# withterm/term

Hardware: AMD Instinct MI355X
Metric: validated rows/sec, 16-col null+range+unique suite (higher is better)
Workload: dtype int64+f64; 1 GPU; 16-col (8 int64 + 8 float64, 12 nullable) null+range+unique suite: completeness x16, min/max/mean x16, uniqueness x2; rows_total=1000000000, rows_per_gpu=1000000000, cols=16, parallelism=row-range shards x1, HSA_ENABLE_IPC_MODE_LEGACY=0, suite_algorithmic_bytes=129500000000, verified=True

## Files before the change

### term_amd/csrc/distinct_state.cpp

```cpp
#include "api_internal.h"

tgx_status distinct_read_counters(tgx_state *st, DistinctState &ds, unsigned long long *out,
                                         tgx_error *err) {
  memset(out, 0, kNumDistinctCounters * sizeof(unsigned long long));
  if (!ds.counters.p) return TGX_OK;
  HIP_TRY(hipMemcpyAsync(out, ds.counters.p, kNumDistinctCounters * sizeof(unsigned long long),
                         hipMemcpyDeviceToHost, st->stream));
  HIP_TRY(hipStreamSynchronize(st->stream));
  return TGX_OK;
}

tgx_status pinned_readback(tgx_state *st, size_t bytes, tgx_error *err) {
  if (bytes <= st->h_pinned_cap) return TGX_OK;
  pinned_free(st->h_pinned, st->h_pinned_cap);
  st->h_pinned = nullptr;
  st->h_pinned_cap = 0;
  const size_t want = std::max<size_t>(bytes + bytes / 2, 4096);
  HIP_TRY(pinned_alloc(&st->h_pinned, want));
  st->h_pinned_cap = want;
  return TGX_OK;
}

namespace {

// ... 587 lines not shown
        ds.range = top - (uint64_t)base + 1;
        use_bitmap = true;
      }
    }
    if (use_bitmap) {
      size_t words = (size_t)(((ds.range + (1u << 20) - 1) >> 20) << 15) + 4;
      ds.bitmap_words = words - 4;
      if (ds.seen.cap < words * 4 && ds.spare_seen.cap >= words * 4) std::swap(ds.seen, ds.spare_seen);
      if (ds.twice.cap < words * 4 && ds.spare_twice.cap >= words * 4) std::swap(ds.twice, ds.spare_twice);
      HIP_TRY(ds.seen.reserve(words * 4));
      HIP_TRY(hipMemsetAsync(ds.seen.p, 0, words * 4, st->stream));
      if (mult) {
        HIP_TRY(ds.twice.reserve(words * 4));
        HIP_TRY(hipMemsetAsync(ds.twice.p, 0, words * 4, st->stream));
      }
      ds.mode = DistinctMode::kBitmap;
      ds.speculative = !ds.has_hint;
      if (ds.speculative && !facts.range_known) {
        ds.remembered = true;
        ds.remembered_lo = lo;
        ds.remembered_hi = hi;
      }
    } else {
      ds.mode = DistinctMode::kHash;
      ds.remembered = false;
    }
  }
  if (ds.mode == DistinctMode::kBitmap && ds.speculative && !ds.partitioned && facts.range_known &&
      !ds.outliers_possible)
    TGX_TRY(bitmap_grow(st, ds, mult, facts.lo, facts.hi, c.length, err));
  if (ds.mode == DistinctMode::kBitmap && ds.speculative) {
    auto u = [](int64_t v) { return (uint64_t)v ^ 0x8000000000000000ull; };
    const bool covered = facts.range_known && u(facts.lo) >= u(ds.base) && u(facts.hi) - u(ds.base) < ds.range;
    if (!covered) ds.outliers_possible = true;
  }
  if (ds.mode == DistinctMode::kBitmap) {
    bitmap_shape(ds, c.length, mult, &prep->sub_bits, &prep->key16, &prep->n_buckets, &prep->partitioned);
    if (ds.partitioned) prep->partitioned = false;
  }
  return TGX_OK;
}

namespace {

tgx_status distinct_run_numeric(tgx_state *st, size_t slot, const tgx_column &c, const NumericPrep &prep,
                                       int stats_slot, tgx_error *err, const tgx_column *orig) {
  const DistinctTask &task = st->plan->distinct[slot];
  const tgx_column &keep = (orig && orig->mem == TGX_MEM_DEVICE && is_widened(orig->type)) ? *orig : c;
  DistinctState &ds = st->distinct[slot];
  const bool mult = task.multiplicity;
  const DistinctColDesc d = numeric_desc(c, mult);
  const uint64_t bytes = (uint64_t)c.length * 8 + (c.validity ? (uint64_t)(c.length + 7) / 8 : 0);
  if (ds.mode == DistinctMode::kUndecided) return TGX_OK;
  if (ds.mode == DistinctMode::kBitmap) {
    if (ds.speculative) ds.retained.push_back(keep);
    if (prep.partitioned) {
      PartitionParams pp;
      memset(&pp, 0, sizeof(pp));
      pp.values = c.values;
      pp.validity = c.validity;
      pp.offset = c.offset;
      pp.length = c.length;
      pp.base = ds.base;
      pp.range = ds.range;
      pp.sub_bits = prep.sub_bits;
      pp.n_buckets = (uint32_t)prep.n_buckets;
      const uint64_t tiles = ((uint64_t)c.length + kPartitionTile - 1) / kPartitionTile;
      pp.bucket0 = 0;
      pp.n_lists = pp.n_buckets;
      if (prep.range_known) {
        auto u = [](int64_t v) { return (uint64_t)v ^ 0x8000000000000000ull; };
        const uint64_t ub = u(ds.base);
        const uint64_t rlo = u(prep.lo) > ub ? u(prep.lo) - ub : 0;
        uint64_t rhi = u(prep.hi) > ub ? u(prep.hi) - ub : 0;
        rhi = std::min(rhi, ds.range - 1);
        if (rlo <= rhi) {
          pp.bucket0 = (uint32_t)(rlo >> pp.sub_bits);
          pp.n_lists = (uint32_t)(rhi >> pp.sub_bits) - pp.bucket0 + 1;
        }
      }
      const char *p20 = getenv("TGX_PACK20");
      const bool no_pack20 = p20 && atoi(p20) == 0;
      const bool pack20 = !prep.key16 && prep.sub_bits <= (mult ? 19u : 20u) && !no_pack20;
      uint64_t cap = (uint64_t)c.length / pp.n_lists;
      cap = cap + cap / 4 + (prep.key16 ? 32 : pack20 ? 24 : 16) * tiles + 4096;
      pp.cap = prep.key16 ? (cap + 31) & ~31ull : pack20 ? (cap + 23) / 24 * 24 : (cap + 15) & ~15ull;
      if (pp.cap >= (1ull << 32) - 64) return fail(err, TGX_INTERNAL, "distinct: list capacity out of range");
      pp.want_multiplicity = mult ? 1 : 0;
      pp.key16 = prep.key16 ? 1 : pack20 ? 2 : 0;
      pp.force_form = ds.remembered_form;
      HIP_TRY(ds.lists.reserve(prep.key16 ? (uint64_t)pp.n_lists * pp.cap * sizeof(uint16_t)
                               : pack20   ? (uint64_t)pp.n_lists * pp.cap / 3 * 8
                                          : (uint64_t)pp.n_lists * pp.cap * sizeof(uint32_t)));
      HIP_TRY(ds.cursors.reserve((2 * pp.n_buckets + 1) * sizeof(unsigned long long)));
      pp.lists = ds.lists.as<uint32_t>();
      pp.cursors = ds.cursors.as<unsigned long long>();
      pp.seen = ds.seen.as<uint32_t>();
      pp.twice = mult ? ds.twice.as<uint32_t>() : nullptr;
      const int grid = partition_grid(c.length, g_ctx.n_cu);
      if (stats_slot >= 0) {
        HIP_TRY(ds.stat_partials.reserve((size_t)(grid + 1) * sizeof(ScanPartial)));
        HIP_TRY(ds.outlier_stats.reserve(sizeof(OutlierStats)));
        pp.stats = ds.stat_partials.as<ScanPartial>();
        pp.outliers = ds.outlier_stats.as<OutlierStats>();
      }
      unsigned long long *cnt = ds.counters.as<unsigned long long>();
      static_assert(kCntDistinct == 0 && kCntTwice == 1, "partition_init_kernel clears the two totals together");
      launch_partition_init(pp, cnt + kCntDistinct, st->stream);
      {
        ProfScope ps(st, "distinct", bytes);
        launch_partition(pp, cnt, g_ctx.n_cu, st->stream);
        HIP_TRY(launch_bucket_apply(pp, cnt, st->stream));
      }
      if (stats_slot >= 0) {
        ScanLaunch L;
        memset(&L, 0, sizeof(L));
        L.cols[0].length = c.length;
        L.cols[0].is_float = 0;
        L.acc_index[0] = stats_slot;
        launch_scan_reduce_only(L, 1, grid, pp.stats, st->d_scan_acc.as<ScanAcc>(), st->stream, pp.outliers);
      }
    } else {
      ProfScope ps(st, "distinct", bytes);
      launch_distinct_bitmap(d, bitmap_view(ds), ds.counters.as<unsigned long long>(), st->stream);
    }
  } else {
    if (ds.fp_staged) TGX_TRY(distinct_resolve(st, slot, err));
    if (ds.capacity == 0 && fp_lists_fit(c)) {
      FpLists l1, l2;
      uint32_t *fb_lo = nullptr;
      TGX_TRY(fp_lists_stage(st, ds, c.length, false, &l1, &l2, &fb_lo, err));
      ProfScope ps(st, "distinct", bytes), ps_lists(st, "distinct_lists", 0);
      launch_key_lists(d, l1, l2, mult ? 1 : 0, ds.fp_per_list.as<uint2>(), ds.counters.as<unsigned long long>(),
                       st->stream);
      ds.retained.push_back(keep);
      return TGX_OK;
    }
    TGX_TRY(hash_ensure(st, ds, mult, (uint64_t)c.length, err));
    ProfScope ps(st, "distinct", bytes);
    launch_distinct_hash(d, hash_view(ds), ds.counters.as<unsigned long long>(), st->stream);
  }
  return TGX_OK;
}

tgx_status retained_numeric_view(tgx_state *st, const tgx_column &col, std::vector<std::unique_ptr<DevBuf>> &tmp,
                                        tgx_column *out, tgx_error *err) {
  *out = col;
  if (!is_widened(col.type)) return TGX_OK;
  const int64_t e0 = col.offset & ~(int64_t)63;
  const int64_t slots = col.offset - e0 + col.length;
  tmp.emplace_back(new DevBuf());
  DevBuf *w = tmp.back().get();
  HIP_TRY(w->reserve((size_t)slots * 8 + 16));
  launch_widen32((const uint8_t *)col.values + narrow_bytes(col.type, e0), w->p, slots, widen_mode(col.type), g_ctx.n_cu,
                 st->stream);
  out->type = widened_type(col.type);
  out->values = w->p;
  out->validity = col.validity ? col.validity + (e0 >> 3) : nullptr;
  out->offset = col.offset - e0;
  return TGX_OK;
}

}

tgx_status distinct_update(tgx_state *st, size_t slot, const tgx_column &c, const BatchKeyFacts &facts,
                           const NumericPrep &prep, tgx_error *err, const std::vector<DictGather> *gathers,
                           int stats_slot, const tgx_column *orig) {
  const DistinctTask &task = st->plan->distinct[slot];
// ... 515 lines not shown
```

### term_amd/csrc/kernels/distinct_types.h

```cpp
#pragma once
#include <stdint.h>

namespace tgx {

constexpr uint64_t kEmptyKey = 0xFFFFFFFFFFFFFFFFULL;

struct DistinctColDesc {
  const void *values;
  const uint8_t *validity;
  int64_t offset;
  int64_t length;
  int32_t want_multiplicity;
  int32_t pad;
};

struct HashSetView {
  uint64_t *keys;
  uint32_t *dup;
  uint64_t mask;
  uint64_t *store;
  unsigned long long *store_cursor;
  uint64_t store_words;
  uint64_t *pending;
  uint32_t *pending_counts;
  uint64_t pending_region;
  uint32_t pending_waves, pad_;
};
inline uint32_t exact_blocks(uint64_t items) {
  uint64_t blocks = (items + 255) / 256;
  if (blocks < 1) blocks = 1;
  if (blocks > 2048) blocks = 2048;
  return (uint32_t)blocks;
}
inline uint32_t exact_waves(uint64_t items) { return exact_blocks(items) * 4; }
inline uint64_t exact_region(uint64_t items) {
  const uint64_t threads = (uint64_t)exact_blocks(items) * 256;
  return (items + threads - 1) / threads * 64;
}

struct FpKey {
  uint32_t k[4], k1[4], k2[4];
};
inline void fp_key_times_two(const uint32_t in[4], uint32_t out[4]) {
  const uint32_t carry = (in[3] >> 31) ? 0x87u : 0u;
  out[3] = (in[3] << 1) | (in[2] >> 31);
  out[2] = (in[2] << 1) | (in[1] >> 31);
  out[1] = (in[1] << 1) | (in[0] >> 31);
  out[0] = (in[0] << 1) ^ carry;
}
inline FpKey fp_key_expand(const uint32_t k[4]) {
  FpKey key;
  for (int i = 0; i < 4; i++) key.k[i] = k[i];
  fp_key_times_two(key.k, key.k1);
  fp_key_times_two(key.k1, key.k2);
  return key;
}

struct Utf8ColDesc {
  const void *offsets;
  const uint8_t *data;
  const uint8_t *validity;
  int64_t offset;
  int64_t length;
  int32_t large_offsets;
  int32_t want_multiplicity;
  const void *views;
  const uint8_t *const *buffers;
  FpKey key;
};

struct BitmapView {
  uint32_t *seen;
  uint32_t *twice;
  int64_t base;
  uint64_t range;
};

constexpr uint32_t kMaxPartitions = 2048;
constexpr uint32_t kListPad = 0xFFFFFFFFu;
constexpr int kRunPad4 = 16, kRunPad2 = 32;
constexpr int kPartitionThreads = 1024;
constexpr int kPartitionKeysPerThread = 32;
constexpr int kPartitionTile = kPartitionThreads * kPartitionKeysPerThread;
constexpr int kSliceWordsLds = 32768;

struct PartitionParams {
  const void *values;
  const uint8_t *validity;
  int64_t offset;
  int64_t length;
  int64_t base;
  uint64_t range;
  uint32_t sub_bits;
  uint32_t n_buckets;
  uint64_t cap;
  uint32_t *lists;
  unsigned long long *cursors;
  uint32_t *seen;
  uint32_t *twice;
  int32_t want_multiplicity;
  int32_t key16;
  struct ScanPartial *stats;
  struct OutlierStats *outliers;
  uint32_t bucket0, n_lists;
  int32_t force_form;
};

struct OutlierStats {
  long long mn, mx;
  unsigned long long lo32_sum;
  long long hi32_sum;
  unsigned long long count;
};

struct DistinctSample {
  int64_t min_v, max_v;
  unsigned long long count;
  unsigned long long pad;
};

struct KeyRecord {
  uint64_t key;
  uint64_t count;
};

struct KeyRecord128 {
  uint64_t a, b;
  uint64_t count;
  uint64_t pad;
};

constexpr int kFpFan = 256;
constexpr int kFpXcds = 8;
constexpr int kFpTile = 2048;
constexpr uint32_t kFpSlots = 4096;
constexpr uint32_t kFpListMax = 24576;
constexpr int64_t kFpMinRows = 1 << 21;
struct FpLists {
  uint64_t *recs;
  uint32_t *offered;
  uint64_t cap;
};

enum {
  kCntDistinct = 0,
  kCntTwice = 1,
  kCntEmptyRows = 2,
  kCntValidRows = 3,
  kCntOutOfRange = 4,
  kCntSpare = 5,
  kCntStoreFull = 6,
  kCntForm = 7,
  kNumDistinctCounters = 8
};

struct TupleCol {
  int32_t kind;
  int32_t dict_large;
  const void *values;
  const void *offsets;
  const uint8_t *data;
  const uint8_t *const *buffers;
  const uint8_t *validity;
  int64_t offset;
  const uint8_t *dict_validity;
  int64_t dict_offset;
};
constexpr int kMaxTupleCols = 8;
struct TupleDesc {
  TupleCol cols[kMaxTupleCols];
  int32_t n_cols;
  int32_t want_multiplicity;
  int64_t length;
  FpKey key;
};

}
```

### term_amd/csrc/kernels/partition.hip

```cpp
#include <hip/hip_runtime.h>

#include <type_traits>

#include "device_types.h"
#include "distinct_types.h"
#include "keyset_device.h"

namespace tgx {

template <int THREADS, int KPT, bool VALIDITY>
__device__ __forceinline__ void partition_load_tile(const PartitionParams &p, int64_t tile, bool wide,
                                                    int64_t (&key)[KPT], uint32_t &ok) {
  constexpr int kPartitionThreads = THREADS;
  constexpr int kTile = kPartitionThreads * KPT;
  global_i64_ptr vals = (global_i64_ptr)(uintptr_t)((const int64_t *)p.values + p.offset);
  global_u8_ptr vbits = VALIDITY ? (global_u8_ptr)(uintptr_t)p.validity : (global_u8_ptr) nullptr;
  const uint32_t tid = threadIdx.x;
  const int64_t row0 = tile * kTile;
  const bool full = row0 + kTile <= p.length;
  ok = 0;
  if (full && wide) {
    typedef long long i64x2 __attribute__((ext_vector_type(2)));
    typedef const i64x2 __attribute__((address_space(1))) *global_i64x2_ptr;
    global_i64x2_ptr pv = (global_i64x2_ptr)(vals + row0) + tid;
    const bool pair_bytes = vbits && (p.offset & 1) == 0;
    ok = (uint32_t)((1ull << KPT) - 1ull);
    if (pair_bytes) {
      uint8_t vb[KPT / 2];
#pragma unroll
      for (int j = 0; j < KPT / 2; j++) {
        const int64_t bit = p.offset + row0 + (int64_t)j * 2 * kPartitionThreads + 2 * tid;
        vb[j] = vbits[bit >> 3];
      }
      ok = 0;
#pragma unroll
      for (int j = 0; j < KPT / 2; j++) {
        const int64_t bit = p.offset + row0 + (int64_t)j * 2 * kPartitionThreads + 2 * tid;
        ok |= (uint32_t)((vb[j] >> (bit & 7)) & 3) << (2 * j);
      }
    } else if (vbits) {
      ok = 0;
#pragma unroll
      for (int j = 0; j < KPT; j++) {
        const int64_t bit = p.offset + row0 + (int64_t)(j / 2) * 2 * kPartitionThreads + 2 * tid + (j & 1);
        ok |= (uint32_t)TGX_VALID_BIT(vbits, bit) << j;
      }
    }
    if (VALIDITY) asm volatile("" : "+v"(ok));
#pragma unroll
    for (int j = 0; j < KPT / 2; j++) {
      i64x2 v = pv[(int64_t)j * kPartitionThreads];
      key[2 * j] = v.x;
      key[2 * j + 1] = v.y;
    }
  } else {
#pragma unroll
    for (int j = 0; j < KPT; j++) {
      const int64_t i = row0 + (int64_t)j * kPartitionThreads + tid;
      const bool in = i < p.length;
      key[j] = vals[in ? i : p.length - 1];
      bool valid = in;
      if (in && vbits) {
        const int64_t bit = p.offset + i;
        valid = TGX_VALID_BIT(vbits, bit);
      }
      ok |= (uint32_t)valid << j;
    }
  }
}

template <int THREADS, int KPT, int MAXP, int PAD, bool KEY16, bool PACK20, bool CLUSTERED, class MidFn, class StoreFn>
__device__ __forceinline__ void partition_process_tile(const PartitionParams &p, uint32_t *sorted, uint32_t *hist,
                                                       uint32_t *toff, uint32_t *gbase, uint32_t *wave_sums,
                                                       uint32_t *long_runs, const uint32_t (&rel)[KPT], uint64_t ok,
                                                       MidFn &&mid,
                                                       StoreFn &&before_stores) {
  constexpr uint32_t NW = THREADS / 64;
  constexpr int BPT = MAXP / THREADS;
  constexpr int NS = MAXP / (NW * 64);
  static_assert(MAXP % THREADS == 0 && MAXP % (NW * 64) == 0 && PAD % 4 == 0, "shape");
  constexpr uint32_t RPAD = PACK20 ? 24u : KEY16 ? (uint32_t)kRunPad2 : (uint32_t)PAD;
  auto pad_up = [](uint32_t h) -> uint32_t { return PACK20 ? (h + 23u) / 24u * 24u : (h + (RPAD - 1u)) & ~(RPAD - 1u); };
  const bool fill = p.want_multiplicity != 0;
  auto pack6 = [&](uint32_t o, uint32_t h, uint32_t i) -> uint4 {
    uint64_t w[2];
    if (!fill) {
#pragma unroll
      for (int q = 0; q < 2; q++) {
        const uint32_t i0 = i + 3u * q;
        const uint64_t a = sorted[o + (i0 < h ? i0 : h - 1)], b = sorted[o + (i0 + 1 < h ? i0 + 1 : h - 1)],
                       c = sorted[o + (i0 + 2 < h ? i0 + 2 : h - 1)];
        w[q] = a | (b << 20) | (c << 40);
      }
    } else {
#pragma unroll
      for (int q = 0; q < 2; q++) {
        uint64_t e[3];
#pragma unroll
        for (uint32_t j = 0; j < 3; j++) {
          const uint32_t at = i + 3u * q + j;
          e[j] = at < h ? (uint64_t)sorted[o + at] : 0xFFFFFull;
        }
        w[q] = e[0] | (e[1] << 20) | (e[2] << 40);
      }
    }
    return make_uint4((uint32_t)w[0], (uint32_t)(w[0] >> 32), (uint32_t)w[1], (uint32_t)(w[1] >> 32));
  };
  const uint32_t tid = threadIdx.x;
  const uint32_t lane = tid & 63, wave = tid >> 6;
  const uint32_t sub_mask = (uint32_t)((1ull << p.sub_bits) - 1);
  for (uint32_t b = tid; b < (uint32_t)MAXP; b += THREADS) hist[b] = 0;
  constexpr uint32_t kLongRun = 1024, kMaxLongRuns = THREADS * KPT / kLongRun;
  if (CLUSTERED && tid == 0) long_runs[kMaxLongRuns] = 0;
  __syncthreads();
  bool whole = false;
  if (CLUSTERED) {
    uint32_t agreed = 0;
#pragma unroll
    for (int j = 0; j < KPT; j++) {
      const bool okj = (ok >> j) & 1;
      const uint32_t b = rel[j] >> p.sub_bits;
      const uint64_t act = __ballot(okj);
      const uint32_t first = act ? (uint32_t)__builtin_ctzll(act) : 0u;
      const uint32_t b0 = (uint32_t)__builtin_amdgcn_readlane((int)b, (int)first);
      agreed |= (__ballot(okj && b != b0) == 0 ? 1u : 0u) << j;
    }
    whole = agreed == (uint32_t)((1ull << KPT) - 1ull);
  }
  if (CLUSTERED && whole) {
#pragma unroll
    for (int j = 0; j < KPT; j++) {
      const uint64_t act = __ballot((ok >> j) & 1);
      const uint32_t first = act ? (uint32_t)__builtin_ctzll(act) : 64u;
      if (lane == first) atomicAdd(&hist[rel[j] >> p.sub_bits], (uint32_t)__builtin_popcountll(act));
    }
  } else {
#pragma unroll
    for (int j = 0; j < KPT; j++)
      if ((ok >> j) & 1) atomicAdd(&hist[rel[j] >> p.sub_bits], 1u);
  }
  __syncthreads();
  {
    uint32_t h[BPT], sum = 0;
#pragma unroll
    for (int k = 0; k < BPT; k++) {
      h[k] = hist[BPT * tid + k];
      sum += h[k];
    }
    uint32_t incl = sum;
#pragma unroll
    for (int d = 1; d < 64; d <<= 1) {
      uint32_t up = __shfl_up(incl, d, 64);
      if (lane >= (uint32_t)d) incl += up;
    }
    if (lane == 63) wave_sums[wave] = incl;
    __syncthreads();
    uint32_t excl = incl - sum;
    for (uint32_t w = 0; w < wave; w++) excl += wave_sums[w];
#pragma unroll
    for (int k = 0; k < BPT; k++) {
      const uint32_t b = BPT * tid + k;
      toff[b] = excl;
      hist[b] = excl;
      uint32_t g = 0;
      if (h[k] && b - p.bucket0 >= p.n_lists) {
        g = 0xFFFFFFFFu;
      } else if (h[k]) {
        const unsigned long long padded = pad_up(h[k]);
        const unsigned long long at = atomicAdd(&p.cursors[b], padded);
        if (at + padded > p.cap) {
          atomicMin(&p.cursors[p.n_buckets + b], at);
          g = 0xFFFFFFFFu;
        } else {
          g = (uint32_t)at;
          if (CLUSTERED && h[k] >= kLongRun) long_runs[atomicAdd(&long_runs[kMaxLongRuns], 1u)] = b;
        }
      }
      gbase[b] = g;
      excl += h[k];
    }
    if (tid == THREADS - 1) toff[MAXP] = excl;
  }
  __syncthreads();
  __builtin_amdgcn_sched_barrier(0);
  mid();
  __builtin_amdgcn_sched_barrier(0);
  if (CLUSTERED && whole) {
#pragma unroll
    for (int j = 0; j < KPT; j++) {
      const bool okj = (ok >> j) & 1;
      const uint64_t act = __ballot(okj);
      const uint32_t first = act ? (uint32_t)__builtin_ctzll(act) : 64u;
      uint32_t at = 0;
      if (lane == first) at = atomicAdd(&hist[rel[j] >> p.sub_bits], (uint32_t)__builtin_popcountll(act));
      at = (uint32_t)__builtin_amdgcn_readlane((int)at, (int)(first & 63u));
      const uint32_t before =
          __builtin_amdgcn_mbcnt_hi((uint32_t)(act >> 32), __builtin_amdgcn_mbcnt_lo((uint32_t)act, 0u));
      if (okj) sorted[at + before] = rel[j] & sub_mask;
    }
  } else {
#pragma unroll
    for (int j = 0; j < KPT; j++) {
      if (!((ok >> j) & 1)) continue;
      const uint32_t pos = atomicAdd(&hist[rel[j] >> p.sub_bits], 1u);
      sorted[pos] = rel[j] & sub_mask;
    }
  }
  __syncthreads();
  __builtin_amdgcn_sched_barrier(0);
  before_stores();
  __builtin_amdgcn_sched_barrier(0);
  {
    uint32_t m_o[NS], m_h[NS], m_g[NS];
#pragma unroll
    for (int s2 = 0; s2 < NS; s2++) {
      const uint32_t b = (lane + 64 * s2) * NW + wave;
      const bool in = b < p.n_buckets;
      const uint32_t o = in ? toff[b] : 0;
      m_o[s2] = o;
      m_h[s2] = in ? toff[b + 1] - o : 0;
      m_g[s2] = in ? gbase[b] : 0;
    }
    const uint32_t n_meta = (p.n_buckets > wave) ? (p.n_buckets - wave + NW - 1) / NW : 0;
    constexpr uint32_t LPB = (KEY16 || PACK20) ? 4u : 16u, BPS = 64u / LPB, KPL = PACK20 ? 6u : KEY16 ? 8u : 4u;
    const uint32_t grp = lane / LPB, sub = lane % LPB;
#pragma unroll
    for (int s2 = 0; s2 < NS; s2++) {
      const uint32_t m_end = n_meta > 64u * s2 ? (n_meta - 64u * s2 < 64u ? n_meta - 64u * s2 : 64u) : 0;
      for (uint32_t m0 = 0; m0 < m_end; m0 += BPS) {
        const uint32_t m = m0 + grp, src = m & 63;
        const uint32_t o = __shfl(m_o[s2], src, 64), g = __shfl(m_g[s2], src, 64);
        uint32_t h = __shfl(m_h[s2], src, 64);
        if (m >= m_end) h = 0;
        if (CLUSTERED && h >= kLongRun && g != 0xFFFFFFFFu) h = 0;
        if (h == 0) continue;
        const uint32_t b = (m + 64 * s2) * NW + wave;
        if (g != 0xFFFFFFFFu) {
          const uint32_t padded = pad_up(h);
          if (PACK20) {
            uint8_t *dst = (uint8_t *)p.lists + ((uint64_t)(b - p.bucket0) * p.cap + g) / 3 * 8;
            for (uint32_t i = KPL * sub; i < padded; i += KPL * LPB) *(uint4 *)(dst + (uint64_t)(i / 3) * 8) = pack6(o, h, i);
          } else if (KEY16) {
            uint16_t *dst = (uint16_t *)p.lists + (uint64_t)(b - p.bucket0) * p.cap + g;
            for (uint32_t i = KPL * sub; i < padded; i += KPL * LPB) {
              uint32_t k8[8];
#pragma unroll
              for (uint32_t j = 0; j < 8; j++) k8[j] = sorted[o + (i + j < h ? i + j : h - 1)];
              uint4 v;
              v.x = k8[0] | (k8[1] << 16);
              v.y = k8[2] | (k8[3] << 16);
              v.z = k8[4] | (k8[5] << 16);
              v.w = k8[6] | (k8[7] << 16);
              *(uint4 *)&dst[i] = v;
            }
          } else {
            uint32_t *dst = p.lists + (uint64_t)(b - p.bucket0) * p.cap + g;
            for (uint32_t i = KPL * sub; i < padded; i += KPL * LPB) {
              uint4 v;
              v.x = i < h ? sorted[o + i] : kListPad;
              v.y = i + 1 < h ? sorted[o + i + 1] : kListPad;
              v.z = i + 2 < h ? sorted[o + i + 2] : kListPad;
              v.w = i + 3 < h ? sorted[o + i + 3] : kListPad;
              *(uint4 *)&dst[i] = v;
            }
          }
        } else {
          for (uint32_t i = sub; i < h; i += LPB) {
            const uint64_t r = ((uint64_t)b << p.sub_bits) | sorted[o + i];
            const uint32_t bit = 1u << (r & 31);
            const uint32_t prev = atomicOr(&p.seen[r >> 5], bit);
            if ((prev & bit) && p.want_multiplicity) atomicOr(&p.twice[r >> 5], bit);
          }
        }
      }
    }
  }
  if (CLUSTERED) {
    const uint32_t n_long = long_runs[kMaxLongRuns];
    for (uint32_t q = 0; q < n_long; q++) {
      const uint32_t b = long_runs[q];
      const uint32_t o = toff[b], h = toff[b + 1] - o, g = gbase[b];
      const uint32_t padded = pad_up(h);
      if (PACK20) {
        uint8_t *dst = (uint8_t *)p.lists + ((uint64_t)(b - p.bucket0) * p.cap + g) / 3 * 8;
        for (uint32_t i = 6u * tid; i < padded; i += 6u * THREADS) *(uint4 *)(dst + (uint64_t)(i / 3) * 8) = pack6(o, h, i);
      } else if (KEY16) {
        uint16_t *dst = (uint16_t *)p.lists + (uint64_t)(b - p.bucket0) * p.cap + g;
        for (uint32_t i = 8u * tid; i < padded; i += 8u * THREADS) {
          uint32_t k8[8];
#pragma unroll
          for (uint32_t j = 0; j < 8; j++) k8[j] = sorted[o + (i + j < h ? i + j : h - 1)];
          uint4 v;
          v.x = k8[0] | (k8[1] << 16);
          v.y = k8[2] | (k8[3] << 16);
          v.z = k8[4] | (k8[5] << 16);
          v.w = k8[6] | (k8[7] << 16);
          *(uint4 *)&dst[i] = v;
        }
      } else {
        uint32_t *dst = p.lists + (uint64_t)(b - p.bucket0) * p.cap + g;
        for (uint32_t i = 4u * tid; i < padded; i += 4u * THREADS) {
          uint4 v;
          v.x = i < h ? sorted[o + i] : kListPad;
          v.y = i + 1 < h ? sorted[o + i + 1] : kListPad;
          v.z = i + 2 < h ? sorted[o + i + 2] : kListPad;
          v.w = i + 3 < h ? sorted[o + i + 3] : kListPad;
          *(uint4 *)&dst[i] = v;
        }
      }
    }
  }
  __syncthreads();
}

template <int G>
__device__ __forceinline__ bool merge_word_group(uint32_t cw, uint32_t &cb) {
  const uint32_t lane = threadIdx.x & 63;
#pragma unroll
  for (int d = 1; d < G; d <<= 1) {
    const uint32_t ow = __shfl_xor(cw, d, 64), ob = __shfl_xor(cb, d, 64);
    if (ow == cw) cb |= ob;
  }
  const uint32_t lead = lane & ~(uint32_t)(G - 1);
  const uint64_t agree = __ballot(cw == (uint32_t)__shfl(cw, (int)lead, 64));
  const bool whole = ((agree >> lead) & ((1ull << G) - 1)) == ((1ull << G) - 1);
  return !whole || lane == lead;
}

template <int KPT>
__device__ __forceinline__ void partition_relative(const PartitionParams &p, const int64_t (&key)[KPT],
                                                   uint32_t (&rel)[KPT], uint32_t &outm) {
  outm = 0;
#pragma unroll
  for (int j = 0; j < KPT; j++) {
    const uint64_t r = (uint64_t)key[j] - (uint64_t)p.base;
    outm |= (r >= p.range ? 1u : 0u) << j;
    rel[j] = (uint32_t)r;
    asm volatile("" : "+v"(rel[j]));
  }
  __builtin_amdgcn_sched_barrier(0);
}

template <int KPT, bool STATS>
__device__ __forceinline__ void partition_relative_plain(const PartitionParams &p, const int64_t (&key)[KPT],
                                                         uint32_t (&rel)[KPT], uint64_t &ok, unsigned long long &n_out) {
#pragma unroll
  for (int j = 0; j < KPT; j++) {
    const uint64_t r = (uint64_t)key[j] - (uint64_t)p.base;
    if (((ok >> j) & 1) && r >= p.range) {
      ok &= ~(1ull << j);
      n_out++;
      if (STATS) {
        const long long k = (long long)key[j];
        atomicMin(&p.outliers->mn, k);
        atomicMax(&p.outliers->mx, k);
        atomicAdd(&p.outliers->lo32_sum, (unsigned long long)((uint64_t)k & 0xFFFFFFFFull));
        atomicAdd((unsigned long long *)&p.outliers->hi32_sum, (unsigned long long)(k >> 32));
        atomicAdd(&p.outliers->count, 1ull);
      }
    }
    rel[j] = (uint32_t)r;
    asm volatile("" : "+v"(rel[j]));
  }
  __builtin_amdgcn_sched_barrier(0);
}

template <int THREADS, int KPT>
__device__ __forceinline__ void partition_outlier_stats(const PartitionParams &p, int64_t tile, bool wide, uint32_t outm,
                                                     OutlierStats *lds_out) {
  constexpr int kTile = THREADS * KPT;
  global_i64_ptr vals = (global_i64_ptr)(uintptr_t)((const int64_t *)p.values + p.offset);
  const int64_t row0 = tile * kTile;
  const bool paired = row0 + kTile <= p.length && wide;
  unsigned long long cnt = 0;
  for (int j = 0; j < KPT; j++) {
    if (!((outm >> j) & 1)) continue;
    const int64_t i = paired ? row0 + (int64_t)(j / 2) * 2 * THREADS + 2 * threadIdx.x + (j & 1)
                             : row0 + (int64_t)j * THREADS + threadIdx.x;
    const long long k = vals[i];
    if (k < *(volatile long long *)&lds_out->mn) atomicMin(&lds_out->mn, k);
    if (k > *(volatile long long *)&lds_out->mx) atomicMax(&lds_out->mx, k);
    atomicAdd(&lds_out->lo32_sum, (unsigned long long)((uint64_t)k & 0xFFFFFFFFull));
    atomicAdd((unsigned long long *)&lds_out->hi32_sum, (unsigned long long)(k >> 32));
    cnt++;
  }
  atomicAdd(&lds_out->count, cnt);
}

template <int THREADS, int KPT, int MAXP, int PAD, bool VALIDITY, bool KEY16, bool STATS, bool FORM_CLUSTERED, bool PACK20 = false>
__global__ __launch_bounds__(THREADS) __attribute__((amdgpu_waves_per_eu(4, 4))) void partition_kernel(
    PartitionParams p, unsigned long long *counters) {
  if ((p.force_form ? p.force_form == 2 : __builtin_amdgcn_readfirstlane((int)p.cursors[2 * p.n_buckets]) != 0) != FORM_CLUSTERED)
    return;
  constexpr int kTile = THREADS * KPT;
  __shared__ uint32_t sorted[kTile];
  __shared__ uint32_t hist[MAXP];
  __shared__ uint32_t toff[MAXP + 1];
  __shared__ uint32_t gbase[MAXP];
  __shared__ uint32_t wave_sums[16];
  __shared__ uint32_t long_runs[kTile / 1024 + 1];
  __shared__ uint32_t t_lo, t_hi;
  const bool wide = (((uintptr_t)p.values + (uintptr_t)p.offset * 8) & 15) == 0;
  unsigned long long n_valid = 0, n_out = 0;
  const int64_t n_tiles = (p.length + kTile - 1) / kTile;
  uint32_t rel[KPT];
  __shared__ uint32_t st_min, st_max;
  __shared__ unsigned long long st_sum, st_cnt;
  __shared__ OutlierStats st_out;
  if (STATS && threadIdx.x == 0) {
    st_min = 0xFFFFFFFFu;
    st_max = 0;
    st_sum = 0;
    st_cnt = 0;
    st_out.mn = INT64_MAX;
    st_out.mx = INT64_MIN;
    st_out.lo32_sum = 0;
    st_out.hi32_sum = 0;
    st_out.count = 0;
  }
  if (STATS) __syncthreads();
  auto tile_loop = [&](auto clustered_tag) __attribute__((always_inline)) {
  constexpr bool CLUSTERED = decltype(clustered_tag)::value;
  for (int64_t tile = blockIdx.x; tile < n_tiles; tile += gridDim.x) {
    uint64_t ok;
    {
      int64_t key[KPT];
      uint32_t ok32 = 0;
      partition_load_tile<THREADS, KPT, VALIDITY>(p, tile, wide, key, ok32);
      ok = ok32;
      n_valid += __builtin_popcountll(ok);
      if (CLUSTERED) {
        uint32_t outm;
        partition_relative<KPT>(p, key, rel, outm);
        outm &= ok32;
        ok = ok32 & ~outm;
        if (__ballot(outm != 0)) {
          n_out += __builtin_popcount(outm);
          if (STATS && outm) partition_outlier_stats<THREADS, KPT>(p, tile, wide, outm, &st_out);
        }
      } else {
        partition_relative_plain<KPT, STATS>(p, key, rel, ok, n_out);
      }
    }
    if (STATS) {
      uint32_t tmin = 0xFFFFFFFFu, tmax = 0;
      unsigned long long tsum = 0;
#pragma unroll
      for (int j = 0; j < KPT; j++) {
        const bool in = (ok >> j) & 1;
        tmin = (in && rel[j] < tmin) ? rel[j] : tmin;
        tmax = (in && rel[j] > tmax) ? rel[j] : tmax;
        tsum += in ? rel[j] : 0u;
      }
      unsigned long long tcnt = __builtin_popcountll(ok);
#pragma unroll
      for (int d = 32; d >= 1; d >>= 1) {
        const uint32_t omin = __shfl_down(tmin, d, 64), omax = __shfl_down(tmax, d, 64);
        tmin = omin < tmin ? omin : tmin;
        tmax = omax > tmax ? omax : tmax;
        tsum += __shfl_down(tsum, d, 64);
        tcnt += __shfl_down(tcnt, d, 64);
      }
      if ((threadIdx.x & 63) == 0 && tcnt) {
        atomicMin(&st_min, tmin);
        atomicMax(&st_max, tmax);
        atomicAdd(&st_sum, tsum);
        atomicAdd(&st_cnt, tcnt);
      }
    }
    if (CLUSTERED && !p.want_multiplicity) {
      if (threadIdx.x == 0) {
        t_lo = 0xFFFFFFFFu;
        t_hi = 0;
      }
      __syncthreads();
      uint32_t lo = 0xFFFFFFFFu, hi = 0;
#pragma unroll
      for (int j = 0; j < KPT; j++) {
        const bool in = (ok >> j) & 1;
        lo = (in && rel[j] < lo) ? rel[j] : lo;
        hi = (in && rel[j] > hi) ? rel[j] : hi;
      }
#pragma unroll
      for (int d = 32; d >= 1; d >>= 1) {
        const uint32_t olo = __shfl_xor(lo, d, 64), ohi = __shfl_xor(hi, d, 64);
        lo = olo < lo ? olo : lo;
        hi = ohi > hi ? ohi : hi;
      }
      if ((threadIdx.x & 63) == 0 && lo <= hi) {
        atomicMin(&t_lo, lo);
        atomicMax(&t_hi, hi);
      }
      __syncthreads();
      const uint32_t tlo = t_lo, thi = t_hi;
      if (tlo > thi) continue;
      const uint32_t w0 = tlo >> 5, nw = (thi >> 5) - w0 + 1;
      if (nw <= (uint32_t)kTile) {
        for (uint32_t w = threadIdx.x; w < nw; w += THREADS) sorted[w] = 0;
        __syncthreads();
#pragma unroll
        for (int j = 0; j < KPT; j += 2) {
          uint32_t cw = 0xFFFFFFFFu, cb = 0;
          if ((ok >> j) & 1) {
            cw = (rel[j] >> 5) - w0;
            cb = 1u << (rel[j] & 31);
          }
          if ((ok >> (j + 1)) & 1) {
            const uint32_t w1 = (rel[j + 1] >> 5) - w0, b1 = 1u << (rel[j + 1] & 31);
            if (w1 == cw) {
              cb |= b1;
            } else {
              if (cb) atomicOr(&sorted[cw], cb);
              cw = w1;
              cb = b1;
            }
          }
          const bool send = merge_word_group<16>(cw, cb);
          if (send && cb) atomicOr(&sorted[cw], cb);
        }
        __syncthreads();
        for (uint32_t w = threadIdx.x; w < nw; w += THREADS) {
          const uint32_t v = sorted[w];
          if (v) atomicOr(&p.seen[w0 + w], v);
        }
        __syncthreads();
        continue;
      }
    }
    partition_process_tile<THREADS, KPT, MAXP, PAD, KEY16, PACK20, CLUSTERED>(p, sorted, hist, toff, gbase, wave_sums, long_runs, rel, ok,
                                                                      [] {}, [] {});
  }
  };
  tile_loop(std::integral_constant<bool, FORM_CLUSTERED>{});
  if (STATS) {
    __syncthreads();
    if (threadIdx.x == 0) {
      ScanPartial out;
      out.min_k = INT64_MAX;
      out.max_k = INT64_MIN;
      out.sum_lo = 0;
      out.sum_hi = 0;
      out.non_null = (int64_t)st_cnt;
      out.sum = out.comp = out.s1 = out.s2 = 0.0;
      if (st_cnt) {
        out.min_k = (int64_t)((uint64_t)p.base + st_min);
        out.max_k = (int64_t)((uint64_t)p.base + st_max);
        const __int128 sum = (__int128)st_sum + (__int128)st_cnt * (__int128)p.base;
        out.sum_lo = (uint64_t)sum;
        out.sum_hi = (int64_t)(sum >> 64);
      }
      p.stats[blockIdx.x] = out;
      if (st_out.count) {
        atomicMin(&p.outliers->mn, st_out.mn);
        atomicMax(&p.outliers->mx, st_out.mx);
        atomicAdd(&p.outliers->lo32_sum, st_out.lo32_sum);
        atomicAdd((unsigned long long *)&p.outliers->hi32_sum, (unsigned long long)st_out.hi32_sum);
        atomicAdd(&p.outliers->count, st_out.count);
      }
    }
  }
  block_add2_any(n_valid, n_out, &counters[kCntValidRows], &counters[kCntOutOfRange]);
}


template <int LDS_WORDS, bool KEY16 = false, bool PACK20 = false>
__global__ __launch_bounds__(kPartitionThreads) void bucket_apply_kernel(PartitionParams p,
                                                                         unsigned long long *counters) {
  __shared__ __attribute__((aligned(16))) uint32_t lds[LDS_WORDS];
  const uint32_t tid = threadIdx.x;
  const uint32_t b = blockIdx.x;
  const uint32_t slice_words = (uint32_t)((1ull << p.sub_bits) >> 5);
  uint32_t *l_seen = lds;
  uint32_t *l_twice = lds + slice_words;
  uint32_t *g_seen = p.seen + (uint64_t)b * slice_words;
  uint32_t *g_twice = p.want_multiplicity ? p.twice + (uint64_t)b * slice_words : nullptr;
  for (uint32_t w = tid * 4; w < slice_words; w += kPartitionThreads * 4) {
    *(uint4 *)&l_seen[w] = *(const uint4 *)&g_seen[w];
    if (g_twice) *(uint4 *)&l_twice[w] = *(const uint4 *)&g_twice[w];
  }
  __syncthreads();
  unsigned long long cnt = p.cursors[b];
  const unsigned long long limit = p.cursors[p.n_buckets + b];
  if (cnt > limit) cnt = limit;
  const bool clustered = p.cursors[2 * p.n_buckets] != 0;
  const uint32_t li = b - p.bucket0;
  if (li >= p.n_lists) cnt = 0;
  if (PACK20) {
    const uint8_t *list = (const uint8_t *)p.lists + (uint64_t)li * p.cap / 3 * 8;
    constexpr uint64_t kStepP = (uint64_t)kPartitionThreads * 6;
    for (uint64_t w0 = (uint64_t)(tid & ~63u) * 6; w0 < cnt; w0 += 4 * kStepP) {
      const uint64_t i0 = w0 + (uint64_t)(tid & 63u) * 6;
      typedef unsigned int u32x4 __attribute__((ext_vector_type(4)));
      u32x4 k4[4];
#pragma unroll
      for (int q = 0; q < 4; q++) {
        const uint64_t i = i0 + q * kStepP;
        k4[q] = u32x4{0, 0, 0, 0};
        if (i < cnt) k4[q] = __builtin_nontemporal_load((const u32x4 *)(list + i / 3 * 8));
      }
#pragma unroll
      for (int q = 0; q < 4; q++) {
        if (i0 + q * kStepP >= cnt) continue;
        const uint64_t w[2] = {(uint64_t)k4[q].x | ((uint64_t)k4[q].y << 32), (uint64_t)k4[q].z | ((uint64_t)k4[q].w << 32)};
#pragma unroll
        for (int u = 0; u < 6; u++) {
          const uint32_t k = (uint32_t)(w[u / 3] >> (20 * (u % 3))) & 0xFFFFFu;
          const uint32_t bit = 1u << (k & 31);
          if (g_twice) {
            if (k == 0xFFFFFu) continue;
            const uint32_t prev = atomicOr(&l_seen[k >> 5], bit);
            if (prev & bit) atomicOr(&l_twice[k >> 5], bit);
          } else {
            atomicOr(&l_seen[k >> 5], bit);
          }
        }
      }
// ... 266 lines not shown
```

Baseline: 42.64 billion rows/s.

## Allocate per-workgroup chunks in partition lists to cut global cursor atomics

Each workgroup now reserves multi-run chunks of list space per bucket and tracks its current and next chunk in LDS. Later tiles append runs into this local chunk instead of doing a global atomicAdd per bucket per tile. A run that does not fit spills into a prefetched or freshly reserved next chunk, with a small overflow table for extra runs. A close-out pass pads any unused chunk space with filler keys. This trades fewer global atomics and better-coalesced list writes for more LDS use, more list capacity, extra padding writes, and considerably more complex placement logic.

After: 40.92 billion rows/s. 0.96x the previous value.

```diff
diff --git a/term_amd/csrc/distinct_state.cpp b/term_amd/csrc/distinct_state.cpp
--- a/term_amd/csrc/distinct_state.cpp
+++ b/term_amd/csrc/distinct_state.cpp
@@ -693,8 +693,16 @@
       const char *p20 = getenv("TGX_PACK20");
       const bool no_pack20 = p20 && atoi(p20) == 0;
       const bool pack20 = !prep.key16 && prep.sub_bits <= (mult ? 19u : 20u) && !no_pack20;
+      const uint64_t run_pad = prep.key16 ? 32 : pack20 ? 24 : 16;
+      const uint64_t n_wg = (uint64_t)partition_grid(c.length, g_ctx.n_cu);
+      const uint64_t runs_per_chunk = std::min<uint64_t>(4, std::max<uint64_t>(1, tiles / n_wg / 16));
+      const uint64_t avg_run = std::min<uint64_t>((uint64_t)c.length, kPartitionTile) / pp.n_lists + run_pad / 2;
+      uint64_t lines = 1;
+      while (lines < 32 && 2 * lines * run_pad <= runs_per_chunk * avg_run + run_pad) lines *= 2;
+      pp.chunk = (uint32_t)(lines * run_pad);
+      pp.chunk_mask = (uint32_t)(lines - 1);
       uint64_t cap = (uint64_t)c.length / pp.n_lists;
-      cap = cap + cap / 4 + (prep.key16 ? 32 : pack20 ? 24 : 16) * tiles + 4096;
+      cap = cap + cap / 4 + run_pad * tiles + 4096 + 2 * (uint64_t)pp.chunk * n_wg;
       pp.cap = prep.key16 ? (cap + 31) & ~31ull : pack20 ? (cap + 23) / 24 * 24 : (cap + 15) & ~15ull;
       if (pp.cap >= (1ull << 32) - 64) return fail(err, TGX_INTERNAL, "distinct: list capacity out of range");
       pp.want_multiplicity = mult ? 1 : 0;
diff --git a/term_amd/csrc/kernels/distinct_types.h b/term_amd/csrc/kernels/distinct_types.h
--- a/term_amd/csrc/kernels/distinct_types.h
+++ b/term_amd/csrc/kernels/distinct_types.h
@@ -95,6 +95,8 @@
   uint32_t n_buckets;
   uint64_t cap;
   uint32_t *lists;
+  uint32_t chunk;
+  uint32_t chunk_mask;
   unsigned long long *cursors;
   uint32_t *seen;
   uint32_t *twice;
diff --git a/term_amd/csrc/kernels/partition.hip b/term_amd/csrc/kernels/partition.hip
--- a/term_amd/csrc/kernels/partition.hip
+++ b/term_amd/csrc/kernels/partition.hip
@@ -69,12 +69,64 @@
   }
 }
 
-template <int THREADS, int KPT, int MAXP, int PAD, bool KEY16, bool PACK20, bool CLUSTERED, class MidFn, class StoreFn>
+constexpr uint32_t kNoChunk = 0xFFFFFFFFu, kListFull = 0xFFFFFFFEu;
+constexpr uint32_t kMaxExtraRuns = 32;
+
+template <uint32_t RPAD>
+__device__ __forceinline__ uint32_t chunk_room(uint32_t c, uint32_t chunk_mask) {
+  const uint32_t used = (c / RPAD) & chunk_mask;
+  return used ? (chunk_mask + 1u - used) * RPAD : 0u;
+}
+template <uint32_t RPAD>
+__device__ __forceinline__ uint32_t whole_chunks(uint32_t need, uint32_t chunk_mask) {
+  return ((need / RPAD + chunk_mask) & ~chunk_mask) * RPAD;
+}
+__device__ __forceinline__ bool outgrows_chunk(uint32_t padded, uint32_t room, uint32_t n, uint32_t chunk) {
+  return n < kListFull && !(n & 1u) && padded > room && padded - room > chunk;
+}
+
+struct RunPlace {
+  uint32_t g0, r, g1m, cur, nxt;
+};
+template <uint32_t RPAD>
+__device__ __forceinline__ RunPlace place_run(const PartitionParams &p, uint32_t b, uint32_t padded, uint32_t c,
+                                              uint32_t n, uint32_t ex) {
+  RunPlace x{kNoChunk, 0u, 0u, c, n};
+  if (b - p.bucket0 >= p.n_lists) return x;
+  const uint32_t room = chunk_room<RPAD>(c, p.chunk_mask);
+  if (padded <= room) {
+    x.g0 = c;
+    x.r = padded;
+    x.cur = c + padded;
+    return x;
+  }
+  uint32_t g1 = kNoChunk;
+  if (n < kListFull && ((n & 1u) || padded - room <= p.chunk)) {
+    g1 = n & ~1u;
+    x.nxt = kNoChunk;
+  } else if (ex != kNoChunk) {
+    g1 = ex;
+  }
+  if (g1 != kNoChunk) {
+    x.g0 = c;
+    x.r = room;
+    x.g1m = g1 - room;
+    x.cur = g1 + (padded - room);
+  }
+  return x;
+}
+__device__ __forceinline__ uint32_t find_extra_run(const uint32_t *extra, uint32_t b) {
+  const uint32_t n = extra[0] < kMaxExtraRuns ? extra[0] : kMaxExtraRuns;
+  for (uint32_t q = 0; q < n; q++)
+    if (extra[1 + 2 * q] == b) return extra[2 + 2 * q];
+  return kNoChunk;
+}
+
+template <int THREADS, int KPT, int MAXP, int PAD, bool KEY16, bool PACK20, bool CLUSTERED>
 __device__ __forceinline__ void partition_process_tile(const PartitionParams &p, uint32_t *sorted, uint32_t *hist,
-                                                       uint32_t *toff, uint32_t *gbase, uint32_t *wave_sums,
-                                                       uint32_t *long_runs, const uint32_t (&rel)[KPT], uint64_t ok,
-                                                       MidFn &&mid,
-                                                       StoreFn &&before_stores) {
+                                                       uint32_t *cur, uint32_t *nxt, uint32_t *wave_sums,
+                                                       uint32_t *long_runs, uint32_t *extra,
+                                                       const uint32_t (&rel)[KPT], uint64_t ok, uint32_t tiles_ahead) {
   constexpr uint32_t NW = THREADS / 64;
   constexpr int BPT = MAXP / THREADS;
   constexpr int NS = MAXP / (NW * 64);
@@ -112,6 +164,7 @@
   for (uint32_t b = tid; b < (uint32_t)MAXP; b += THREADS) hist[b] = 0;
   constexpr uint32_t kLongRun = 1024, kMaxLongRuns = THREADS * KPT / kLongRun;
   if (CLUSTERED && tid == 0) long_runs[kMaxLongRuns] = 0;
+  if (tid == 0) extra[0] = 0;
   __syncthreads();
   bool whole = false;
   if (CLUSTERED) {
@@ -140,6 +193,8 @@
       if ((ok >> j) & 1) atomicAdd(&hist[rel[j] >> p.sub_bits], 1u);
   }
   __syncthreads();
+  uint32_t ahead_b = kNoChunk;
+  unsigned long long ahead_at = 0;
   {
     uint32_t h[BPT], sum = 0;
 #pragma unroll
@@ -157,34 +212,64 @@
     __syncthreads();
     uint32_t excl = incl - sum;
     for (uint32_t w = 0; w < wave; w++) excl += wave_sums[w];
+    const uint32_t chunk = p.chunk;
+    uint32_t want[BPT], slot[BPT];
+    unsigned long long at[BPT];
 #pragma unroll
     for (int k = 0; k < BPT; k++) {
-      const uint32_t b = BPT * tid + k;
-      toff[b] = excl;
+      uint32_t b = BPT * tid + k;
+      asm volatile("" : "+v"(b));
       hist[b] = excl;
-      uint32_t g = 0;
-      if (h[k] && b - p.bucket0 >= p.n_lists) {
-        g = 0xFFFFFFFFu;
-      } else if (h[k]) {
-        const unsigned long long padded = pad_up(h[k]);
-        const unsigned long long at = atomicAdd(&p.cursors[b], padded);
-        if (at + padded > p.cap) {
-          atomicMin(&p.cursors[p.n_buckets + b], at);
-          g = 0xFFFFFFFFu;
-        } else {
-          g = (uint32_t)at;
-          if (CLUSTERED && h[k] >= kLongRun) long_runs[atomicAdd(&long_runs[kMaxLongRuns], 1u)] = b;
-        }
-      }
-      gbase[b] = g;
       excl += h[k];
-    }
-    if (tid == THREADS - 1) toff[MAXP] = excl;
+      want[k] = 0;
+      slot[k] = 0;
+      if (h[k] && b - p.bucket0 < p.n_lists) {
+        const uint32_t padded = pad_up(h[k]), room = chunk_room<RPAD>(cur[b], p.chunk_mask), n = nxt[b];
+        if (padded > room && n == kNoChunk) {
+          want[k] = whole_chunks<RPAD>(padded - room, p.chunk_mask);
+        } else if (outgrows_chunk(padded, room, n, chunk)) {
+          slot[k] = atomicAdd(&extra[0], 1u);
+          if (slot[k] < kMaxExtraRuns) {
+            extra[1 + 2 * slot[k]] = b;
+            extra[2 + 2 * slot[k]] = kNoChunk;
+            want[k] = whole_chunks<RPAD>(padded - room, p.chunk_mask);
+          }
+        } else if (!CLUSTERED && n == kNoChunk && ahead_b == kNoChunk && room - padded < padded * tiles_ahead) {
+          ahead_b = b;
+        }
+      }
+    }
+#pragma unroll
+    for (int k = 0; k < BPT; k++)
+      if (want[k]) at[k] = atomicAdd(&p.cursors[BPT * tid + k], (unsigned long long)want[k]);
+    if (ahead_b != kNoChunk) ahead_at = atomicAdd(&p.cursors[ahead_b], (unsigned long long)chunk);
+#pragma unroll
+    for (int k = 0; k < BPT; k++) {
+      uint32_t b = BPT * tid + k;
+      asm volatile("" : "+v"(b));
+      if (want[k]) {
+        const bool full = at[k] + want[k] > p.cap;
+        if (full) atomicMin(&p.cursors[p.n_buckets + b], at[k]);
+        if (nxt[b] == kNoChunk)
+          nxt[b] = full ? kListFull : ((uint32_t)at[k] | 1u);
+        else if (!full)
+          extra[2 + 2 * slot[k]] = (uint32_t)at[k];
+      }
+      if (CLUSTERED && h[k] >= kLongRun) {
+        const uint32_t padded = pad_up(h[k]), c = cur[b], n = nxt[b];
+        const uint32_t ex = outgrows_chunk(padded, chunk_room<RPAD>(c, p.chunk_mask), n, chunk) ? find_extra_run(extra, b) : kNoChunk;
+        const RunPlace x = place_run<RPAD>(p, b, padded, c, n, ex);
+        if (x.g0 != kNoChunk) {
+          const uint32_t q = atomicAdd(&long_runs[kMaxLongRuns], 1u);
+          long_runs[q] = b;
+          long_runs[kMaxLongRuns + 1 + q] = x.g0;
+          long_runs[2 * kMaxLongRuns + 1 + q] = x.r;
+          long_runs[3 * kMaxLongRuns + 1 + q] = x.g1m;
+        }
+      }
+    }
   }
   __syncthreads();
-  __builtin_amdgcn_sched_barrier(0);
-  mid();
-  __builtin_amdgcn_sched_barrier(0);
   if (CLUSTERED && whole) {
 #pragma unroll
     for (int j = 0; j < KPT; j++) {
@@ -206,70 +291,100 @@
       sorted[pos] = rel[j] & sub_mask;
     }
   }
+  if (ahead_b != kNoChunk) {
+    if (ahead_at + p.chunk > p.cap) {
+      atomicMin(&p.cursors[p.n_buckets + ahead_b], ahead_at);
+      nxt[ahead_b] = kListFull;
+    } else {
+      nxt[ahead_b] = (uint32_t)ahead_at;
+    }
+  }
   __syncthreads();
-  __builtin_amdgcn_sched_barrier(0);
-  before_stores();
-  __builtin_amdgcn_sched_barrier(0);
+  constexpr uint32_t LPB = (KEY16 || PACK20) ? 4u : 16u, BPS = 64u / LPB, KPL = PACK20 ? 6u : KEY16 ? 8u : 4u;
+  auto store_run = [&](uint32_t b, uint32_t o, uint32_t h, uint32_t g0, uint32_t r, uint32_t g1m, uint32_t first,
+                       uint32_t step) {
+    const uint32_t padded = pad_up(h);
+    const uint64_t base = (uint64_t)(b - p.bucket0) * p.cap;
+    if (PACK20) {
+      uint8_t *dst = (uint8_t *)p.lists + base / 3 * 8;
+      for (uint32_t i = first; i < padded; i += step) {
+        const uint32_t e = (i < r ? g0 : g1m) + i;
+        *(uint4 *)(dst + (uint64_t)(e / 3) * 8) = pack6(o, h, i);
+      }
+    } else if (KEY16) {
+      uint16_t *dst = (uint16_t *)p.lists + base;
+      for (uint32_t i = first; i < padded; i += step) {
+        uint32_t k8[8];
+#pragma unroll
+        for (uint32_t j = 0; j < 8; j++) k8[j] = sorted[o + (i + j < h ? i + j : h - 1)];
+        uint4 v;
+        v.x = k8[0] | (k8[1] << 16);
+        v.y = k8[2] | (k8[3] << 16);
+        v.z = k8[4] | (k8[5] << 16);
+        v.w = k8[6] | (k8[7] << 16);
+        *(uint4 *)&dst[(i < r ? g0 : g1m) + i] = v;
+      }
+    } else {
+      uint32_t *dst = p.lists + base;
+      for (uint32_t i = first; i < padded; i += step) {
+        uint4 v;
+        v.x = i < h ? sorted[o + i] : kListPad;
+        v.y = i + 1 < h ? sorted[o + i + 1] : kListPad;
+        v.z = i + 2 < h ? sorted[o + i + 2] : kListPad;
+        v.w = i + 3 < h ? sorted[o + i + 3] : kListPad;
+        *(uint4 *)&dst[(i < r ? g0 : g1m) + i] = v;
+      }
+    }
+  };
   {
-    uint32_t m_o[NS], m_h[NS], m_g[NS];
+    uint32_t m_o[NS], m_h[NS], m_g0[NS], m_r[NS], m_g1m[NS];
 #pragma unroll
     for (int s2 = 0; s2 < NS; s2++) {
-      const uint32_t b = (lane + 64 * s2) * NW + wave;
+      uint32_t b = (lane + 64 * s2) * NW + wave;
+      asm volatile("" : "+v"(b));
       const bool in = b < p.n_buckets;
-      const uint32_t o = in ? toff[b] : 0;
+      const uint32_t o = (in && b) ? hist[b - 1] : 0;
+      const uint32_t h = in ? hist[b] - o : 0;
       m_o[s2] = o;
-      m_h[s2] = in ? toff[b + 1] - o : 0;
-      m_g[s2] = in ? gbase[b] : 0;
+      m_h[s2] = h;
+      m_g0[s2] = kNoChunk;
+      m_r[s2] = 0;
+      m_g1m[s2] = 0;
+      if (h) {
+        const uint32_t padded = pad_up(h), c = cur[b], n = nxt[b];
+        const uint32_t ex = outgrows_chunk(padded, chunk_room<RPAD>(c, p.chunk_mask), n, p.chunk) ? find_extra_run(extra, b) : kNoChunk;
+        const RunPlace x = place_run<RPAD>(p, b, padded, c, n, ex);
+        m_g0[s2] = x.g0;
+        m_r[s2] = x.r;
+        m_g1m[s2] = x.g1m;
+        if (x.g0 != kNoChunk) {
+          cur[b] = x.cur;
+          if (x.nxt != n) nxt[b] = x.nxt;
+        }
+      }
     }
     const uint32_t n_meta = (p.n_buckets > wave) ? (p.n_buckets - wave + NW - 1) / NW : 0;
-    constexpr uint32_t LPB = (KEY16 || PACK20) ? 4u : 16u, BPS = 64u / LPB, KPL = PACK20 ? 6u : KEY16 ? 8u : 4u;
     const uint32_t grp = lane / LPB, sub = lane % LPB;
 #pragma unroll
     for (int s2 = 0; s2 < NS; s2++) {
       const uint32_t m_end = n_meta > 64u * s2 ? (n_meta - 64u * s2 < 64u ? n_meta - 64u * s2 : 64u) : 0;
       for (uint32_t m0 = 0; m0 < m_end; m0 += BPS) {
         const uint32_t m = m0 + grp, src = m & 63;
-        const uint32_t o = __shfl(m_o[s2], src, 64), g = __shfl(m_g[s2], src, 64);
+        const uint32_t o = __shfl(m_o[s2], src, 64), g0 = __shfl(m_g0[s2], src, 64), r = __shfl(m_r[s2], src, 64),
+                       g1m = __shfl(m_g1m[s2], src, 64);
         uint32_t h = __shfl(m_h[s2], src, 64);
         if (m >= m_end) h = 0;
-        if (CLUSTERED && h >= kLongRun && g != 0xFFFFFFFFu) h = 0;
+        if (CLUSTERED && h >= kLongRun && g0 != kNoChunk) h = 0;
         if (h == 0) continue;
         const uint32_t b = (m + 64 * s2) * NW + wave;
-        if (g != 0xFFFFFFFFu) {
-          const uint32_t padded = pad_up(h);
-          if (PACK20) {
-            uint8_t *dst = (uint8_t *)p.lists + ((uint64_t)(b - p.bucket0) * p.cap + g) / 3 * 8;
-            for (uint32_t i = KPL * sub; i < padded; i += KPL * LPB) *(uint4 *)(dst + (uint64_t)(i / 3) * 8) = pack6(o, h, i);
-          } else if (KEY16) {
-            uint16_t *dst = (uint16_t *)p.lists + (uint64_t)(b - p.bucket0) * p.cap + g;
-            for (uint32_t i = KPL * sub; i < padded; i += KPL * LPB) {
-              uint32_t k8[8];
-#pragma unroll
-              for (uint32_t j = 0; j < 8; j++) k8[j] = sorted[o + (i + j < h ? i + j : h - 1)];
-              uint4 v;
-              v.x = k8[0] | (k8[1] << 16);
-              v.y = k8[2] | (k8[3] << 16);
-              v.z = k8[4] | (k8[5] << 16);
-              v.w = k8[6] | (k8[7] << 16);
-              *(uint4 *)&dst[i] = v;
-            }
-          } else {
-            uint32_t *dst = p.lists + (uint64_t)(b - p.bucket0) * p.cap + g;
-            for (uint32_t i = KPL * sub; i < padded; i += KPL * LPB) {
-              uint4 v;
-              v.x = i < h ? sorted[o + i] : kListPad;
-              v.y = i + 1 < h ? sorted[o + i + 1] : kListPad;
-              v.z = i + 2 < h ? sorted[o + i + 2] : kListPad;
-              v.w = i + 3 < h ? sorted[o + i + 3] : kListPad;
-              *(uint4 *)&dst[i] = v;
-            }
-          }
+        if (g0 != kNoChunk) {
+          store_run(b, o, h, g0, r, g1m, KPL * sub, KPL * LPB);
         } else {
           for (uint32_t i = sub; i < h; i += LPB) {
-            const uint64_t r = ((uint64_t)b << p.sub_bits) | sorted[o + i];
-            const uint32_t bit = 1u << (r & 31);
-            const uint32_t prev = atomicOr(&p.seen[r >> 5], bit);
-            if ((prev & bit) && p.want_multiplicity) atomicOr(&p.twice[r >> 5], bit);
+            const uint64_t rr = ((uint64_t)b << p.sub_bits) | sorted[o + i];
+            const uint32_t bit = 1u << (rr & 31);
+            const uint32_t prev = atomicOr(&p.seen[rr >> 5], bit);
+            if ((prev & bit) && p.want_multiplicity) atomicOr(&p.twice[rr >> 5], bit);
           }
         }
       }
@@ -279,38 +394,51 @@
     const uint32_t n_long = long_runs[kMaxLongRuns];
     for (uint32_t q = 0; q < n_long; q++) {
       const uint32_t b = long_runs[q];
-      const uint32_t o = toff[b], h = toff[b + 1] - o, g = gbase[b];
-      const uint32_t padded = pad_up(h);
-      if (PACK20) {
-        uint8_t *dst = (uint8_t *)p.lists + ((uint64_t)(b - p.bucket0) * p.cap + g) / 3 * 8;
-        for (uint32_t i = 6u * tid; i < padded; i += 6u * THREADS) *(uint4 *)(dst + (uint64_t)(i / 3) * 8) = pack6(o, h, i);
-      } else if (KEY16) {
-        uint16_t *dst = (uint16_t *)p.lists + (uint64_t)(b - p.bucket0) * p.cap + g;
-        for (uint32_t i = 8u * tid; i < padded; i += 8u * THREADS) {
-          uint32_t k8[8];
-#pragma unroll
-          for (uint32_t j = 0; j < 8; j++) k8[j] = sorted[o + (i + j < h ? i + j : h - 1)];
-          uint4 v;
-          v.x = k8[0] | (k8[1] << 16);
-          v.y = k8[2] | (k8[3] << 16);
-          v.z = k8[4] | (k8[5] << 16);
-          v.w = k8[6] | (k8[7] << 16);
-          *(uint4 *)&dst[i] = v;
-        }
-      } else {
-        uint32_t *dst = p.lists + (uint64_t)(b - p.bucket0) * p.cap + g;
-        for (uint32_t i = 4u * tid; i < padded; i += 4u * THREADS) {
-          uint4 v;
-          v.x = i < h ? sorted[o + i] : kListPad;
-          v.y = i + 1 < h ? sorted[o + i + 1] : kListPad;
-          v.z = i + 2 < h ? sorted[o + i + 2] : kListPad;
-          v.w = i + 3 < h ? sorted[o + i + 3] : kListPad;
-          *(uint4 *)&dst[i] = v;
-        }
-      }
+      const uint32_t o = b ? hist[b - 1] : 0, h = hist[b] - o;
+      store_run(b, o, h, long_runs[kMaxLongRuns + 1 + q], long_runs[2 * kMaxLongRuns + 1 + q],
+                long_runs[3 * kMaxLongRuns + 1 + q], KPL * tid, KPL * THREADS);
     }
   }
   __syncthreads();
+}
+
+template <int THREADS, int PAD, bool KEY16, bool PACK20>
+__device__ __forceinline__ void partition_close_chunks(const PartitionParams &p, const uint32_t *cur, const uint32_t *nxt) {
+  constexpr uint32_t RPAD = PACK20 ? 24u : KEY16 ? (uint32_t)kRunPad2 : (uint32_t)PAD;
+  __threadfence();
+  __syncthreads();
+  for (uint32_t b = threadIdx.x; b < p.n_buckets; b += THREADS) {
+    const uint32_t c = cur[b], n = nxt[b];
+    if (c == 0) continue;
+    const uint32_t room = chunk_room<RPAD>(c, p.chunk_mask), ahead = n < kListFull ? p.chunk : 0u, n0 = n & ~1u;
+    if (room + ahead == 0) continue;
+    const uint64_t base = (uint64_t)(b - p.bucket0) * p.cap;
+    if (PACK20) {
+      uint8_t *dst = (uint8_t *)p.lists + base / 3 * 8;
+      uint64_t w = 0x0FFFFFFFFFFFFFFFull;
+      if (!p.want_multiplicity) {
+        const uint64_t last = __hip_atomic_load((const uint64_t *)(dst + (uint64_t)((c - 1) / 3) * 8), __ATOMIC_RELAXED,
+                                                __HIP_MEMORY_SCOPE_AGENT);
+        const uint64_t k = (last >> (20 * ((c - 1) % 3))) & 0xFFFFFull;
+        w = k | (k << 20) | (k << 40);
+      }
+      const uint4 v = make_uint4((uint32_t)w, (uint32_t)(w >> 32), (uint32_t)w, (uint32_t)(w >> 32));
+      for (uint32_t i = 0; i < room; i += 6) *(uint4 *)(dst + (uint64_t)((c + i) / 3) * 8) = v;
+      for (uint32_t i = 0; i < ahead; i += 6) *(uint4 *)(dst + (uint64_t)((n0 + i) / 3) * 8) = v;
+    } else if (KEY16) {
+      uint16_t *dst = (uint16_t *)p.lists + base;
+      const uint32_t k = __hip_atomic_load(&dst[c - 1], __ATOMIC_RELAXED, __HIP_MEMORY_SCOPE_AGENT);
+      const uint32_t kk = k | (k << 16);
+      const uint4 v = make_uint4(kk, kk, kk, kk);
+      for (uint32_t i = 0; i < room; i += 8) *(uint4 *)&dst[c + i] = v;
+      for (uint32_t i = 0; i < ahead; i += 8) *(uint4 *)&dst[n0 + i] = v;
+    } else {
+      uint32_t *dst = p.lists + base;
+      const uint4 v = make_uint4(kListPad, kListPad, kListPad, kListPad);
+      for (uint32_t i = 0; i < room; i += 4) *(uint4 *)&dst[c + i] = v;
+      for (uint32_t i = 0; i < ahead; i += 4) *(uint4 *)&dst[n0 + i] = v;
+    }
+  }
 }
 
 template <int G>
@@ -395,10 +523,16 @@
   constexpr int kTile = THREADS * KPT;
   __shared__ uint32_t sorted[kTile];
   __shared__ uint32_t hist[MAXP];
-  __shared__ uint32_t toff[MAXP + 1];
-  __shared__ uint32_t gbase[MAXP];
+  __shared__ uint32_t cur[MAXP];
+  __shared__ uint32_t nxt[MAXP];
   __shared__ uint32_t wave_sums[16];
-  __shared__ uint32_t long_runs[kTile / 1024 + 1];
+  __shared__ uint32_t long_runs[4 * (kTile / 1024) + 1];
+  __shared__ uint32_t extra[2 * kMaxExtraRuns + 1];
+  for (uint32_t b = threadIdx.x; b < (uint32_t)MAXP; b += THREADS) {
+    cur[b] = 0;
+    nxt[b] = kNoChunk;
+  }
+  __syncthreads();
   __shared__ uint32_t t_lo, t_hi;
   const bool wide = (((uintptr_t)p.values + (uintptr_t)p.offset * 8) & 15) == 0;
   unsigned long long n_valid = 0, n_out = 0;
@@ -527,11 +661,13 @@
         continue;
       }
     }
-    partition_process_tile<THREADS, KPT, MAXP, PAD, KEY16, PACK20, CLUSTERED>(p, sorted, hist, toff, gbase, wave_sums, long_runs, rel, ok,
-                                                                      [] {}, [] {});
+    const int64_t ahead = (n_tiles - 1 - tile) / gridDim.x;
+    partition_process_tile<THREADS, KPT, MAXP, PAD, KEY16, PACK20, CLUSTERED>(p, sorted, hist, cur, nxt, wave_sums, long_runs, extra, rel,
+                                                                      ok, (uint32_t)(ahead < 64 ? ahead : 64));
   }
   };
   tile_loop(std::integral_constant<bool, FORM_CLUSTERED>{});
+  partition_close_chunks<THREADS, PAD, KEY16, PACK20>(p, cur, nxt);
   if (STATS) {
     __syncthreads();
     if (threadIdx.x == 0) {
```
